# atenpas/gpd

Measured on NVIDIA H100. Metric: grasp candidates/sec end-to-end (15ch), higher is better.
Workload: dtype f64 geometry / f32 LeNet

## Files before the change

### gpd_b200/csrc/api.cu

```cuda
#include <atomic>
#include <cfloat>
#include <cmath>
#include <cstdarg>
#include <cstdio>
#include <cstdlib>
#include <cstring>
#include <string>
#include <vector>

#include "common.cuh"

static char g_create_err[512] = "";

struct StageTimes {
  struct Span { int stage; cudaEvent_t b, e; };
  std::vector<cudaEvent_t> pool;
  size_t used = 0;
  std::vector<Span> spans;
  cudaEvent_t get() {
    if (used == pool.size()) {
      cudaEvent_t e;
      cudaEventCreate(&e);
      pool.push_back(e);
    }
// ... 2117 lines not shown
        const int c = st.ecount[(size_t)r * B + b];
        if (eval_round_counts_out) eval_round_counts_out[(size_t)b * R + r] = c;
        if (eval_xyz_out) memcpy(eval_xyz_out + 3 * o, ev.data() + 3 * ((size_t)b * R + r) * S, sizeof(double) * 3 * c);
        o += c;
      }
      if (eval_offsets_out) eval_offsets_out[b + 1] = (int32_t)o;
    }
  }
  if (kept_offsets_out) memcpy(kept_offsets_out, st.koff.data(), sizeof(int32_t) * ((size_t)B + 1));
  if (kept_xyz_out)
    for (int b = 0; b < B; b++)
      memcpy(kept_xyz_out + 3 * (size_t)st.koff[b], kp.data() + 3 * ((size_t)st.init_off[b] + (size_t)b * RS),
             sizeof(double) * 3 * (size_t)(st.koff[b + 1] - st.koff[b]));
  return B;
}

void gpdb_free_result(gpdb_result *r) {
  if (!r) return;
  if (r->owner_) {
    HostArena *a = (HostArena *)r->owner_;
    a->in_use = false;
    arena_unref(a);
  } else {
    free(r->frame_valid);
    free(r->frames);
    free(r->pose_flags);
    free(r->pose_scores);
    free(r->candidates);
    free(r->images);
  }
  memset(r, 0, sizeof(*r));
}

int gpdb_debug_phase_cycles(gpdb_ctx *ctx, int enable, uint64_t cycles_out[16]) {
  if (!ctx) return GPDB_ERR_INVALID;
  CUDA_TRY(cudaSetDevice(ctx->device));
  CUDA_TRY(cudaStreamSynchronize(ctx->stream));
  if (ctx->d_prof && cycles_out)
    CUDA_TRY(cudaMemcpy(cycles_out, ctx->d_prof, sizeof(uint64_t) * 16, cudaMemcpyDeviceToHost));
  if (enable && !ctx->d_prof) CUDA_TRY(cudaMalloc(&ctx->d_prof, sizeof(uint64_t) * 32));
  if (enable) CUDA_TRY(cudaMemset(ctx->d_prof, 0, sizeof(uint64_t) * 32));
  if (!enable && ctx->d_prof) {
    cudaFree(ctx->d_prof);
    ctx->d_prof = nullptr;
  }
  return GPDB_OK;
}

int gpdb_debug_path_counts(gpdb_ctx *ctx, uint64_t counts_out[16]) {
  if (!ctx || !counts_out) return GPDB_ERR_INVALID;
  CUDA_TRY(cudaSetDevice(ctx->device));
  CUDA_TRY(cudaStreamSynchronize(ctx->stream));
  if (ctx->d_prof)
    CUDA_TRY(cudaMemcpy(counts_out, ctx->d_prof + GPDB_PROF_PATH, sizeof(uint64_t) * 16, cudaMemcpyDeviceToHost));
  else
    memset(counts_out, 0, sizeof(uint64_t) * 16);
  return GPDB_OK;
}

int gpdb_last_timings(const gpdb_ctx *ctx, double ms_out[8]) {
  if (!ctx || !ms_out) return GPDB_ERR_INVALID;
  for (int i = 0; i < 8; i++) ms_out[i] = ctx->last_ms[i];
  return GPDB_OK;
}

}
```

### gpd_b200/csrc/common.cuh

```cuda
#pragma once
#include <cuda_runtime.h>
#include <stdint.h>

#include "../../include/gpd_b200.h"
#include "../../include/gpd_b200_shadow.h"

#define GPDB_MAX_ORIENT 32
#define GPDB_MAX_SLOTS 32
#define GPDB_MAX_DEEPEN 64
#define GPDB_MAX_NSP 128

struct DevParams {
  double finger_width, hand_outer_diameter, hand_depth, hand_height, init_bite;
  int P, n_axes, n_orient, nfp;
  int axes[GPDB_MAX_HAND_AXES];
  int deepen, slots_disjoint, all_axes_z;
  double inv_slot_step;
  double fs[GPDB_MAX_SLOTS];
  double fsw[GPDB_MAX_SLOTS];
  int J;
  double topj[GPDB_MAX_DEEPEN], botj[GPDB_MAX_DEEPEN];
  double cosf;
  int min_viable;
  double min_ap, max_ap, ws[6];
// ... 41 lines not shown
struct CloudTable {
  const CloudDesc *d;
  const int *soff;
  int n;
};

struct CloudSet {
  float4 *pts4;
  float *xyz;
  double *nrm;
  uint8_t *cam;
  int *src;
  int *cell_start;
  CloudDesc *desc;
  int *soff;
  int *off;
  int *sel;
  int *pos;
  size_t point_cap, cell_cap, desc_cap;
  int n, maxk;
  bool has_src;
  double *samples;
  int n_samples;
  size_t samples_cap;
  int positions(int b) const { return n_samples ? pos[b + 1] - pos[b] : 0; }
  DevCloud view;
  int points() const { return n ? off[n] : 0; }
  CloudTable table() const { return CloudTable{desc, soff, n}; }
};

#define GPDB_NERR 8

#define GPDB_PROF_PATH 16
enum PathEvent {
  PATH_FRAMES_T1, PATH_FRAMES_T2, PATH_HANDS_T2, PATH_HANDS_T3, PATH_HANDS_SLAB, PATH_IMG2_BOX, PATH_IMG2_NONUNIT, PATH_IMG_GL,
  PATH_IMG2_CAST, PATH_IMG2_DRAW, PATH_IMG2_STASH, PATH_IMG_CAST, PATH_IMG_DRAW, PATH_IMG_STASH, PATH_IMG_BALL
};

#define CUDA_TRY(expr)                                                                        \
  do {                                                                                        \
    cudaError_t e__ = (expr);                                                                 \
    if (e__ != cudaSuccess) {                                                                 \
      gpdb_set_error(ctx, GPDB_ERR_CUDA, "%s:%d %s -> %s", __FILE__, __LINE__, #expr,         \
                     cudaGetErrorString(e__));                                                \
      return GPDB_ERR_CUDA;                                                                   \
    }                                                                                         \
  } while (0)

struct LenetWeights {
  float *c1w, *c1b, *c2w, *c2b, *i1w, *i1b, *i2w, *i2b;
  int C;
  bool set;
};

struct C1Affine {
  float scale[20], bias[20];
};
struct LenetTc {
  void *b1, *b2, *b3;
  C1Affine c1_aff;
  int npl, nch1;
  float w2_scale, a2_scale, w3_scale, x3_scale;
  bool ready;
};

struct StageTimes;
// ... 165 lines not shown
```

### gpd_b200/csrc/geometry.cu

```cuda
#include <cfloat>
#include <climits>
#include <cstdlib>
#include <vector>
#include <cub/cub.cuh>

#include "common.cuh"
#include "grid.cuh"

namespace {

constexpr int NT_HANDS = 256;
#ifndef GPDB_NT_IMG
#define GPDB_NT_IMG 512
#endif
constexpr int NT_IMG = GPDB_NT_IMG;
constexpr int LRF_WARPS = 4;
constexpr int LRF_CAP_GLOBAL = 16384;
constexpr int LRF_CAP = 1024;
constexpr int BOX_CAP = 2048;
constexpr int MAXPIX = 64 * 64;

__device__ __forceinline__ void to_frame(const double *F, double v0, double v1, double v2, double &o0, double &o1,
                                         double &o2) {
  o0 = (F[0] * v0 + F[1] * v1) + F[2] * v2;
// ... 1152 lines not shown
  }
  return !__any_sync(0xffffffffu, empty);
}
template <int NT>
__device__ __forceinline__ void occ_ballot(unsigned *occf, int t, bool occupied) {
  const unsigned word = __ballot_sync(0xffffffffu, occupied);
  if ((threadIdx.x & 31) == 0) occf[(threadIdx.x >> 5) + t * (NT / 32)] = word;
}

template <int NT>
__device__ __noinline__ float dilated_min(const float *F, int S) {
  float mn = FLT_MAX;
  for (int pix = threadIdx.x; pix < S * S; pix += NT) {
    const int r = pix / S, c = pix - r * S;
    float m = -FLT_MAX;
    for (int dr = -1; dr <= 1; dr++)
      for (int dc = -1; dc <= 1; dc++) {
        const int rr = r + dr, cc = c + dc;
        if (rr >= 0 && rr < S && cc >= 0 && cc < S) m = fmaxf(m, F[rr * S + cc]);
      }
    mn = fminf(mn, m);
  }
  return mn;
}

#define PHASE(i)                                                        \
  do {                                                                  \
    if (prof && threadIdx.x == 0) {                                     \
      long long now__ = clock64();                                      \
      if ((i) > 1) atomicAdd(prof + (i), (unsigned long long)(now__ - t_phase)); \
      t_phase = now__;                                                  \
    }                                                                   \
  } while (0)


__device__ __forceinline__ int warp_append(bool pred, int *counter) {
  const unsigned mk = __ballot_sync(0xffffffffu, pred);
  if (!mk) return 0;
  const int lane = threadIdx.x & 31, leader = __ffs(mk) - 1;
  int base = 0;
  if (lane == leader) base = atomicAdd(counter, __popc(mk));
  base = __shfl_sync(0xffffffffu, base, leader);
  return base + __popc(mk & ((1u << lane) - 1));
}

template <class R, class E>
__device__ __forceinline__ void warp_expand_bits(unsigned bits, unsigned code, R &&reserve, E &&emit) {
  const int lane = threadIdx.x & 31;
  const int cnt = __popc(bits);
  int incl = cnt;
#pragma unroll
  for (int o = 1; o < 32; o <<= 1) {
    const int v = __shfl_up_sync(0xffffffffu, incl, o);
    if (lane >= o) incl += v;
  }
  const int total = __shfl_sync(0xffffffffu, incl, 31);
  const int base = reserve(total);
  for (int j0 = 0; j0 < total; j0 += 32) {
    const int j = j0 + lane;
    int w = 0;
#pragma unroll
    for (int s = 16; s; s >>= 1) {
      const int v = __shfl_sync(0xffffffffu, incl, w + s - 1);
      if (v <= j) w += s;
    }
    const unsigned wbits = __shfl_sync(0xffffffffu, bits, w), wcode = __shfl_sync(0xffffffffu, code, w);
    const int wexcl = __shfl_sync(0xffffffffu, incl - cnt, w);
    if (j < total) emit(base + j, wcode | __fns(wbits, 0, j - wexcl + 1));
  }
}

template <class E>
__device__ __forceinline__ void expand_bitmap(const unsigned *bitmap, int nbits, int d1, int *counter, E &&emit) {
  const int lane = threadIdx.x & 31;
  for (int wd0 = 0; wd0 * 32 < nbits; wd0 += NT_IMG) {
    const int wd = wd0 + threadIdx.x;
    const unsigned bits = (wd * 32 < nbits) ? bitmap[wd] : 0u;
    const int rowi = wd >> 1;
    const unsigned code = ((unsigned)(rowi % d1) << 8) | ((unsigned)(rowi / d1) << 16) | ((unsigned)(wd & 1) << 5);
    warp_expand_bits(
        bits, code,
// ... 189 lines not shown
  bool nrm, dep;
};
template <class W>
__device__ __forceinline__ void winners_to_planes(const PointPlanes &pp, const float (&mnv)[2], const float (&mxv)[2],
                                                  bool background, W &&for_each_winner) {
  const Quant qn(mnv[0], mxv[0]), qd(mnv[1], mxv[1]);
  if (background) {
    const unsigned bg_n = qn(0.0f) * 0x01010101u, bg_d = qd(0.0f) * 0x01010101u;
    for (int k = threadIdx.x; k < (pp.plb >> 2); k += NT_IMG) {
      if (pp.nrm)
#pragma unroll
        for (int c = 0; c < 3; c++) reinterpret_cast<unsigned *>(pp.base + (size_t)(pp.cb + c) * pp.plb)[k] = bg_n;
      if (pp.dep) reinterpret_cast<unsigned *>(pp.base + (size_t)pp.cd * pp.plb)[k] = bg_d;
    }
    __syncthreads();
  }
  for_each_winner([&](int o, float n0, float n1, float n2, float dv) {
    if (pp.nrm) {
      pp.base[(size_t)(pp.cb + 0) * pp.plb + o] = (uint8_t)qn(n0);
      pp.base[(size_t)(pp.cb + 1) * pp.plb + o] = (uint8_t)qn(n1);
      pp.base[(size_t)(pp.cb + 2) * pp.plb + o] = (uint8_t)qn(n2);
    }
    if (pp.dep) pp.base[(size_t)pp.cd * pp.plb + o] = (uint8_t)qd(dv);
  });
}


template <class Sm, class G>
__device__ __noinline__ void shadow_setup(const DevParams &P, const G &Gd, Sm &sm, double gmax, unsigned *bitmap,
                                             int bm_total) {
  const gpdb_pose &h = sm.h;
  const int tid = threadIdx.x;
  const double voxel = GPDB_SHADOW_VOXEL;
  if (tid == 0) {
    const double jmax = gmax * voxel * 0.3 + 1e-9;
    const double half_od = P.vol_w / 2.0;
    double mn[3] = {DBL_MAX, DBL_MAX, DBL_MAX}, mx[3] = {-DBL_MAX, -DBL_MAX, -DBL_MAX};
    for (int cr = 0; cr < 8; cr++) {
      double cx = (cr & 1) ? h.bottom + P.vol_d : h.bottom;
      double cy = (cr & 2) ? h.center + half_od : h.center - half_od;
      double cz = (cr & 4) ? P.vol_h : -P.vol_h;
      for (int r = 0; r < 3; r++) {
        double wv = h.frame[r] * cx + h.frame[3 + r] * cy + h.frame[6 + r] * cz + h.sample[r];
        mn[r] = fmin(mn[r], wv);
        mx[r] = fmax(mx[r], wv);
      }
    }
    for (int r = 0; r < 3; r++) {
      int lo = (int)floor((mn[r] - jmax) * P.vox_mult) - 1;
      int hi = (int)floor((mx[r] + jmax) * P.vox_mult) + 1;
      sm.bm_org[r] = lo;
      sm.bm_dims[r] = min(hi - lo + 1, P.bm_dim);
    }
    for (int e = 0; e < 9; e++) sm.fR[e] = (float)h.frame[e];
    for (int r = 0; r < 3; r++) sm.fs[r] = (float)h.sample[r];
    const float jm = (float)(gmax * voxel * 0.3 * 1.7320508075688772 + 2e-5);
    sm.fbx_lo[0] = (float)h.bottom - jm;
    sm.fbx_lo[1] = (float)(h.center - P.vol_w / 2.0) - jm;
    sm.fbx_lo[2] = (float)(-P.vol_h) - jm;
    sm.fbx_hi[0] = (float)(h.bottom + P.vol_d) + jm;
    sm.fbx_hi[1] = (float)(h.center + P.vol_w / 2.0) + jm;
    sm.fbx_hi[2] = (float)P.vol_h + jm;
    const double wm = 0.0105;
    const double bx_lo[3] = {h.bottom - wm, h.center - P.vol_w / 2.0 - wm, -P.vol_h - wm};
    const double bx_hi[3] = {h.bottom + P.vol_d + wm, h.center + P.vol_w / 2.0 + wm, P.vol_h + wm};
    for (int a = 0; a < 3; a++) {
      sm.cull_lo[a] = (float)bx_lo[a] - 1e-5f;
      sm.cull_hi[a] = (float)bx_hi[a] + 1e-5f;
    }
  }
  if (tid < Gd.K) {
    double s0 = sm.center[0] - Gd.vp[tid][0], s1 = sm.center[1] - Gd.vp[tid][1], s2 = sm.center[2] - Gd.vp[tid][2];
    double nn = sqrt((s0 * s0 + s1 * s1) + s2 * s2);
    sm.sv[tid][0] = P.shadow_length * s0 / nn;
    sm.sv[tid][1] = P.shadow_length * s1 / nn;
    sm.sv[tid][2] = P.shadow_length * s2 / nn;
    double svh[3];
    to_frame(h.frame, sm.sv[tid][0], sm.sv[tid][1], sm.sv[tid][2], svh[0], svh[1], svh[2]);
    for (int a = 0; a < 3; a++) {
      const float dv = (float)svh[a];
      sm.cull_inv[tid][a] = fabsf(dv) < 1e-6f ? 0.0f : 1.0f / dv;
    }
  }
  for (int k = tid; k < bm_total; k += NT_IMG) bitmap[k] = 0u;
}

struct VoxelBox {
  int o0, o1, o2, d0, d1, d2;
  template <class Sm>
  __device__ __forceinline__ explicit VoxelBox(const Sm &sm)
      : o0(sm.bm_org[0]), o1(sm.bm_org[1]), o2(sm.bm_org[2]), d0(sm.bm_dims[0]), d1(sm.bm_dims[1]), d2(sm.bm_dims[2]) {}
};

__device__ __forceinline__ bool voxel_point_in_box(const DevParams &P, const gpdb_pose &h, const double *qtab, int v0, int v1,
                                                   int v2, double &x, double &y, double &z) {
  const double voxel = GPDB_SHADOW_VOXEL;
  double g = qtab[gpdb_voxel_hash(v0, v1, v2) & (GPDB_QTAB_SIZE - 1)];
  double jit = 1.0 * g * voxel * 0.3;
  double w0 = (double)v0 * voxel + jit, w1 = (double)v1 * voxel + jit, w2 = (double)v2 * voxel + jit;
  to_frame(h.frame, w0 - h.sample[0], w1 - h.sample[1], w2 - h.sample[2], x, y, z);
  return in_image_box(P, h, x, y, z);
}
// ... 32 lines not shown
  float tmin = 0.0f, tmax = 1.0f;
  bool hit = true;
#pragma unroll
  for (int a = 0; a < 3; a++) {
    if (cull_inv[a] == 0.0f) {
      hit = hit && o3[a] >= sm.cull_lo[a] && o3[a] <= sm.cull_hi[a];
    } else {
      const float t1 = (sm.cull_lo[a] - o3[a]) * cull_inv[a], t2 = (sm.cull_hi[a] - o3[a]) * cull_inv[a];
      tmin = fmaxf(tmin, fminf(t1, t2));
      tmax = fminf(tmax, fmaxf(t1, t2));
    }
  }
  if (!hit || tmin > tmax) return false;
  const int r0 = max((int)floorf(tmin * 32767.0f) - 1, 0), r1 = min((int)ceilf(tmax * 32767.0f) + 1, 32767);
  rg = (unsigned)r0 | ((unsigned)r1 << 16);
  return true;
}

struct CastLists {
  float4 *wl;
  unsigned *wrange;
  int wl_cap;
  unsigned *dlist;
  int dl_cap;
  int path_cast, path_draw;
};

template <class Sm, class G, class BallAt>
__device__ __forceinline__ void cast_camera(const DevParams &P, const G &Gd, const DevCloud &cl, const SegRange &sr,
                                            const float (&q)[3], Sm &sm, const VoxelBox &vb, int k, unsigned *bm,
                                            const CastLists &L, bool use_ball, int nball, BallAt &&ball_at,
                                            unsigned long long *prof, bool count_walks) {
  const int tid = threadIdx.x;
  __syncthreads();
  if (tid == 0) {
    sm.wl_n = 0;
    sm.dl_n = 0;
  }
  __syncthreads();
  auto append = [&](bool ok, const float4 &p, unsigned rg) {
    const int pos = warp_append(ok, &sm.wl_n);
    if (!ok) return;
    const unsigned seed0 = gpdb_shadow_seed((unsigned)sm.h.sample_index, (unsigned)__float_as_int(p.w), (unsigned)k);
    if (pos < L.wl_cap) {
      L.wl[pos] = make_float4(p.x, p.y, p.z, __uint_as_float(seed0));
      L.wrange[pos] = rg;
    } else {
      unsigned seed = seed0;
      const int r0 = (int)(rg & 0xFFFFu), r1 = (int)(rg >> 16);
      for (int t = 0; t < P.nsp; t++) {
        int r = (int)gpdb_fastrand(&seed);
        if (r >= r0 && r <= r1) set_bit(bm, draw_bit(P, sm, vb, (double)p.x, (double)p.y, (double)p.z, seed, k));
      }
    }
  };
  if (use_ball) {
    for (int i0 = 0; i0 < nball; i0 += NT_IMG) {
      const int i = i0 + tid;
      float4 p = make_float4(0.f, 0.f, 0.f, 0.f);
      unsigned rg = 0;
      bool ok = false;
      if (i < nball) {
        p = __ldg(cl.pts4 + ball_at(i));
        ok = cull(sm, k, p, rg);
      }
      append(ok, p, rg);
    }
  } else {
    scan_balanced<NT_IMG>(Gd, cl, sr, sm.seg, [&](bool in, const float4 &p, int) {
      unsigned rg = 0;
      const bool ok = in && l2_simple(q, p.x, p.y, p.z) < P.r2_img && cull(sm, k, p, rg);
      append(ok, p, rg);
    });
    if (count_walks && prof && tid == 0) atomicAdd(prof + 14, 1ull);
  }
  __syncthreads();
  const int nw = min(sm.wl_n, L.wl_cap);
  if (prof && tid == 0) {
    atomicAdd(prof + 9, (unsigned long long)nw);
    if (sm.wl_n > L.wl_cap) atomicAdd(prof + GPDB_PROF_PATH + L.path_cast, (unsigned long long)(sm.wl_n - L.wl_cap));
  }
  const int nsp = P.nsp;
  const unsigned nsp_magic = nsp > 1 ? (unsigned)((0x100000000ull + (unsigned)nsp - 1) / (unsigned)nsp) : 0u;
  const int nd = nw * nsp;
  for (int w0 = 0; w0 < nd; w0 += NT_IMG) {
    const int w = w0 + tid;
    bool pass = false;
    unsigned code = 0, seed = 0;
    if (w < nd) {
      const int item = nsp > 1 ? (int)__umulhi((unsigned)w, nsp_magic) : w, t = w - item * nsp;
      seed = sm.lcgA[t] * __float_as_uint(L.wl[item].w) + sm.lcgC[t];
      const unsigned rg = L.wrange[item];
      const int r = (int)((seed >> 16) & 0x7FFFu);
      pass = r >= (int)(rg & 0xFFFFu) && r <= (int)(rg >> 16);
      code = ((unsigned)item << 7) | (unsigned)t;
    }
    const int pos = warp_append(pass, &sm.dl_n);
    if (pass) {
      if (pos < L.dl_cap) L.dlist[pos] = code;
      else {
        const float4 e = L.wl[code >> 7];
        set_bit(bm, draw_bit(P, sm, vb, (double)e.x, (double)e.y, (double)e.z, seed, k));
      }
    }
  }
  __syncthreads();
  const int ndl = min(sm.dl_n, L.dl_cap);
  if (prof && tid == 0) {
    atomicAdd(prof + 10, (unsigned long long)sm.dl_n);
    if (sm.dl_n > L.dl_cap) atomicAdd(prof + GPDB_PROF_PATH + L.path_draw, (unsigned long long)(sm.dl_n - L.dl_cap));
  }
  auto list_bit = [&](int i) -> int {
    if (i >= ndl) return -1;
    const unsigned code = L.dlist[i];
    const float4 e = L.wl[code >> 7];
    const int t = (int)(code & 127u);
    const unsigned seed = sm.lcgA[t] * __float_as_uint(e.w) + sm.lcgC[t];
    return draw_bit(P, sm, vb, (double)e.x, (double)e.y, (double)e.z, seed, k);
  };
  for (int i = tid; i < ndl; i += 2 * NT_IMG) {
    const int bit_a = list_bit(i), bit_b = list_bit(i + NT_IMG);
    set_bit(bm, bit_a);
    set_bit(bm, bit_b);
  }
}

__device__ __forceinline__ void intersect_bitmaps(unsigned *bitmap, int bm_words, int K, int cam_set) {
  if (K < 2) return;
  for (int wd = threadIdx.x; wd < bm_words; wd += NT_IMG) {
    unsigned acc = bitmap[wd];
    for (int k = 1; k < K; k++)
      if ((cam_set >> k) & 1) acc &= bitmap[(size_t)k * bm_words + wd];
    bitmap[wd] = acc;
  }
}

__device__ __forceinline__ uint2 eval_voxel(const DevParams &P, const gpdb_pose &h, const double *qtab, const double (&inv)[3],
                                            int S, const VoxelBox &vb, unsigned long long *tiles, unsigned code, int pj_lo,
                                            int pj_hi) {
  int b0 = code & 255, b1 = (code >> 8) & 255, b2 = code >> 16;
  double x, y, z;
  if (!voxel_point_in_box(P, h, qtab, b0 + vb.o0, b1 + vb.o1, b2 + vb.o2, x, y, z)) return make_uint2(0u, 0u);
  double u[3];
  int cellv[3];
  unit_cells(P, h, inv, S, x, y, z, u, cellv);
  uint2 st = make_uint2(0u, 0u);
#pragma unroll
  for (int pj = 0; pj < 3; pj++) {
    const Proj pr(pj);
    const int pix = (S - 1 - cellv[pr.a0]) * S + cellv[pr.a1];
    const unsigned qv = unit_q32(u[pr.a2]);
    if (pj >= pj_lo && pj < pj_hi) cell_add(tiles + (size_t)(pj - pj_lo) * S * S + pix, qv);
    if (pj == 2) st = make_uint2((unsigned)pix | 0x80000000u, qv);
  }
  return st;
}

template <class Sm>
__device__ __forceinline__ void shadow_channel(Sm &sm, const double *rcp, int S, unsigned long long *tile, uint8_t *plane,
                                               int rs) {
  constexpr int PIXT = (MAXPIX + NT_IMG - 1) / NT_IMG;
  const int tid = threadIdx.x, SS = S * S;
  float avgr[PIXT];
  unsigned occm = 0;
  float mm[2] = {-FLT_MAX, -FLT_MAX};
#pragma unroll
  for (int t = 0; t < PIXT; t++) {
    const int pix = tid + t * NT_IMG;
    avgr[t] = 0.0f;
    bool oc = false;
    if (pix < SS) {
      const unsigned long long acc = tile[pix];
      const unsigned cntc = (unsigned)(acc >> 48);
      if (cntc) {
        avgr[t] = (float)cell_mean(acc, rcp);
        occm |= 1u << t;
        oc = true;
        mm[0] = fmaxf(mm[0], avgr[t]);
        mm[1] = fmaxf(mm[1], -avgr[t]);
      }
    }
    if (t * NT_IMG < SS) occ_ballot<NT_IMG>(sm.occf, t, oc);
  }
  bool covered;
  block_max<NT_IMG, 2>(mm, sm.fred, sm.occf, S, &covered);
// ... 291 lines not shown
      const int nset = min(sm.wl_n, BL_CAP);
      if (prof && tid == 0) {
        atomicAdd(prof + 11, (unsigned long long)sm.wl_n);
        atomicAdd(prof + 12, (unsigned long long)bn);
        atomicAdd(prof + 13, (unsigned long long)sm.n_img);
        if (sm.wl_n > BL_CAP) atomicAdd(prof + GPDB_PROF_PATH + PATH_IMG_STASH, 1ull);
        if (sm.ball_n > BALL_CAP) atomicAdd(prof + GPDB_PROF_PATH + PATH_IMG_BALL, 1ull);
      }
      for (int i = tid; i < nset; i += NT_IMG) eval_voxel(P, h, qtab, inv, S, vb, tileA, blist[i], 0, 3);
      __syncthreads();
      PHASE(6);
      for (int pj = 0; pj < 3; pj++) shadow_channel(sm, rcp, S, tileA + (size_t)pj * SS, planes + (size_t)(pj * 5 + 4) * PLB, RS);
      __syncthreads();
      for (int k = tid; k < MAXPIX / 32; k += NT_IMG) sm.occf[k] = 0u;
    }
    __syncthreads();
    PHASE(7);
    dilate_assemble(S, RS >> 2, C, [&](int ch) { return planes + (size_t)ch * PLB; }, reinterpret_cast<uint4 *>(p16) + (size_t)b * SS);
    PHASE(8);
  }
}

constexpr int BOX_CAP2 = 1024;
constexpr int IMG2_S = 60;
constexpr int BALL_CAP2 = (IMG2_S * IMG2_S * 16 - 12 * IMG2_S * IMG2_S) / 4;
using Img2Smem = ImgSmemT<2>;
constexpr size_t IMG2_DYN_SMEM = (size_t)2 * 8 * IMG2_S * IMG2_S + (size_t)3 * IMG2_S * IMG2_S + (size_t)BOX_CAP2 * 36;
static_assert(2 * (IMG2_DYN_SMEM + sizeof(Img2Smem) + 1024) <= 228 * 1024, "k_images2 no longer fits two CTAs per SM");

template <bool BATCH>
__global__ void __launch_bounds__(NT_IMG, 2) k_images2(const DevParams *Pp, DevCloud cl0, CloudTable tab, const gpdb_pose *cand, int nc,
                                                       uint8_t *p16, const double *qtab, int *ovf, int *ovf_count,
                                                       unsigned long long *prof) {
  long long t_phase = 0;
  const DevParams &P = *Pp;
  extern __shared__ __align__(16) unsigned char dyn[];
  __shared__ Img2Smem sm;
  constexpr int S = IMG2_S, SS = S * S, RW = S / 4, PLB = SS;
  constexpr int JW = (BOX_CAP2 + NT_IMG - 1) / NT_IMG;
  const int C = P.C;
  unsigned long long *tileA = reinterpret_cast<unsigned long long *>(dyn);
  unsigned long long *tileB = tileA + SS;
  uint8_t *splanes = reinterpret_cast<uint8_t *>(tileB + SS);
  unsigned char *lbase = splanes + 3 * PLB;
  constexpr int LIST_BYTES = BOX_CAP2 * 36;
  const BoxList bl(lbase, BOX_CAP2);
  unsigned *bitmap = reinterpret_cast<unsigned *>(lbase);
  uint8_t *tplanes = reinterpret_cast<uint8_t *>(tileA);
  const int tid = threadIdx.x;
  const int nproj = (C >= 12) ? 3 : 1;
  const bool do_nrm = C != 1, do_dep = C == 1 || C >= 12;
  const int npp = (C == 15 || C == 12) ? 12 : C;
  img_cta_init(sm, P);

  for (int b = blockIdx.x; b < nc; b += gridDim.x) {
    img_begin(sm, cand + b);
    uint8_t *gimg = p16 + (size_t)b * SS * 16;
    int *ball = reinterpret_cast<int *>(gimg + 12 * PLB);
    for (int k = tid; k < (npp * PLB) >> 4; k += NT_IMG) reinterpret_cast<uint4 *>(gimg)[k] = make_uint4(0, 0, 0, 0);
    for (int k = tid; k < SS; k += NT_IMG) reinterpret_cast<uint4 *>(tileA)[k] = make_uint4(0, 0, 0, 0);
    for (int k = tid; k < (3 * PLB) >> 4; k += NT_IMG) reinterpret_cast<uint4 *>(splanes)[k] = make_uint4(0, 0, 0, 0);
    __syncthreads();
    PHASE(1);
    const gpdb_pose &h = sm.h;
    const auto &G = CloudSel<BATCH>::get(tab, h.sample_slot);
    const DevCloud cl = CloudSel<BATCH>::local(G, cl0);
    const double inv[3] = {1.0 / P.vol_d, 1.0 / P.vol_w, 1.0 / (2.0 * P.vol_h)};
// ... 65 lines not shown
        for (int j = 0; j < JW; j++)
          if (wpix[j] >= 0) emit(wpix[j], wv[j][0], wv[j][1], wv[j][2], wv[j][3]);
      });
      if (covered) {
        for (int k = tid; k < SS; k += NT_IMG) reinterpret_cast<uint4 *>(tileA)[k] = make_uint4(0, 0, 0, 0);
        for (int k = tid; k < MAXPIX / 32; k += NT_IMG) sm.occf[k] = 0u;
      } else {
        __syncthreads();
        wipe_cells(bl, bn, S, pr, tileA, tileB, sm.occf);
      }
      __syncthreads();
    }
    PHASE(3);

    if (C == 15) {
      const int K = G.K, bm_words = 2 * P.bm_dim * P.bm_dim;
      shadow_setup(P, G, sm, qtab[GPDB_QTAB_SIZE - 1], bitmap, bm_words * K);
      __syncthreads();
      PHASE(4);
      const VoxelBox vb(sm);
      const int cam_set = sm.cam_or, nball = sm.ball_n;
      float4 *wl = reinterpret_cast<float4 *>(tileA);
      constexpr int WL_CAP = (SS * 8) / 20;
      const CastLists L = {wl, reinterpret_cast<unsigned *>(wl + WL_CAP), WL_CAP, reinterpret_cast<unsigned *>(tileB), 2 * SS,
                           PATH_IMG2_CAST, PATH_IMG2_DRAW};
      for (int k = 0; k < K; k++) {
        if (!((cam_set >> k) & 1)) continue;
        cast_camera(P, G, cl, sr, q, sm, vb, k, bitmap + (size_t)k * bm_words, L, nball <= BALL_CAP2, nball,
                    [&](int i) { return __ldcg(ball + i); },
                    prof, true);
      }
      __syncthreads();
      PHASE(5);
      intersect_bitmaps(bitmap, bm_words, K, cam_set);
      for (int k = tid; k < SS; k += NT_IMG) reinterpret_cast<uint4 *>(tileA)[k] = make_uint4(0, 0, 0, 0);
      if (tid == 0) sm.wl_n = 0;
      __syncthreads();
      const int nbits = 64 * vb.d1 * vb.d2;
      uint2 *stash = reinterpret_cast<uint2 *>(bitmap + (((size_t)bm_words * (K > 1 ? K : 1) + 1) & ~(size_t)1));
      const int ST_CAP = (LIST_BYTES - (int)((reinterpret_cast<unsigned char *>(stash)) - lbase)) / 8;
      expand_bitmap(bitmap, nbits, vb.d1, &sm.wl_n, [&](int pos, unsigned code) {
        if (pos < ST_CAP) stash[pos].x = code;
        else eval_voxel(P, h, qtab, inv, S, vb, tileA, code, 0, 2);
      });
      __syncthreads();
      const int nset_all = sm.wl_n, nset = min(nset_all, ST_CAP);
      if (prof && tid == 0) {
        atomicAdd(prof + 11, (unsigned long long)nset_all);
        atomicAdd(prof + 12, (unsigned long long)bn);
        atomicAdd(prof + 13, (unsigned long long)sm.n_img);
        if (nset_all > ST_CAP) atomicAdd(prof + GPDB_PROF_PATH + PATH_IMG2_STASH, 1ull);
      }
      for (int i = tid; i < nset; i += NT_IMG) stash[i] = eval_voxel(P, h, qtab, inv, S, vb, tileA, stash[i].x, 0, 2);
      __syncthreads();
      PHASE(6);
      shadow_channel(sm, rcp, S, tileA, splanes, S);
      shadow_channel(sm, rcp, S, tileB, splanes + PLB, S);
      __syncthreads();
      for (int k = tid; k < SS / 2; k += NT_IMG) reinterpret_cast<uint4 *>(tileA)[k] = make_uint4(0, 0, 0, 0);
      __syncthreads();
      if (nset_all <= ST_CAP) {
        for (int i = tid; i < nset; i += NT_IMG) {
          const uint2 st = stash[i];
          if (st.x & 0x80000000u) {
            const bool carry = cell_add(tileA + (st.x & 0x7fffffffu), st.y);
            if (prof && carry) atomicAdd(prof + 0, 1ull);
          }
        }
      } else {
        expand_bitmap(bitmap, nbits, vb.d1, nullptr, [&](int, unsigned code) { eval_voxel(P, h, qtab, inv, S, vb, tileA, code, 2, 3); });
      }
      __syncthreads();
      if (prof) {
        unsigned most = 0;
        for (int k = tid; k < SS; k += NT_IMG) most = max(most, (unsigned)(tileA[k] >> 48));
        most = __reduce_max_sync(0xffffffffu, most);
        if ((tid & 31) == 0 && most) atomicMax(prof + 1, (unsigned long long)most);
      }
      shadow_channel(sm, rcp, S, tileA, splanes + 2 * PLB, S);
      __syncthreads();
      for (int k = tid; k < MAXPIX / 32; k += NT_IMG) sm.occf[k] = 0u;
    }
    __syncthreads();
    PHASE(7);
    for (int k = tid; k < (npp * PLB) >> 4; k += NT_IMG)
      reinterpret_cast<uint4 *>(tplanes)[k] = __ldcg(reinterpret_cast<const uint4 *>(gimg) + k);
    __syncthreads();
    dilate_assemble(S, RW, C, [&](int ch) {
      return (C == 15) ? ((ch % 5 == 4) ? splanes + (size_t)(ch / 5) * PLB : tplanes + (size_t)(4 * (ch / 5) + ch % 5) * PLB)
                       : tplanes + (size_t)ch * PLB;
    }, reinterpret_cast<uint4 *>(gimg));
    PHASE(8);
  }
}

__global__ void k_p16_to_hwc(const uint8_t *__restrict__ p16, size_t npix, int C, uint8_t *__restrict__ hwc) {
  const size_t i = (size_t)blockIdx.x * blockDim.x + threadIdx.x;
  if (i >= npix * (size_t)C) return;
  const size_t pix = i / C;
  hwc[i] = p16[pix * 16 + (i - pix * C)];
}
__global__ void k_hwc_to_p16(const uint8_t *__restrict__ hwc, size_t npix, int C, uint8_t *__restrict__ p16) {
  const size_t i = (size_t)blockIdx.x * blockDim.x + threadIdx.x;
  if (i >= npix) return;
  unsigned w[4] = {0u, 0u, 0u, 0u};
  for (int c = 0; c < C; c++) w[c >> 2] |= (unsigned)hwc[i * C + c] << (8 * (c & 3));
  reinterpret_cast<uint4 *>(p16)[i] = make_uint4(w[0], w[1], w[2], w[3]);
}

__global__ void k_batch_desc(const int *bounds, CloudDesc *d, int B, long long *ncell) {
  const int b = blockIdx.x * blockDim.x + threadIdx.x;
  if (b >= B) return;
  CloudDesc &D = d[b];
  float lo[3], hi[3];
  for (int a = 0; a < 3; a++) {
    const int mn = bounds[6 * b + a], mx = bounds[6 * b + 3 + a];
// ... 435 lines not shown
```

### gpd_b200/lib.py

```python
import ctypes as C
import os

import numpy as np

from . import abi

_HERE = os.path.dirname(os.path.abspath(__file__))
SO_PATH = os.environ.get("GPD_B200_LIB") or os.path.join(_HERE, "libgpd_b200.so")
_LIB = None

EXPORTS = [
    "gpdb_params_default", "gpdb_create", "gpdb_destroy", "gpdb_last_error", "gpdb_load_weights_dir",
    "gpdb_set_weights", "gpdb_set_cloud", "gpdb_detect", "gpdb_frames", "gpdb_hand_search", "gpdb_images",
    "gpdb_classify", "gpdb_free_result", "gpdb_last_timings", "gpdb_build_info", "gpdb_detect_resident",
    "gpdb_set_stream", "gpdb_debug_phase_cycles", "gpdb_preprocess_params_default", "gpdb_preprocess",
    "gpdb_get_cloud", "gpdb_get_cloud_source_index", "gpdb_preprocess_timings", "gpdb_detect_select", "gpdb_load_weights_file", "gpdb_read_weights_file", "gpdb_set_samples",
    "gpdb_comm_unique_id", "gpdb_comm_init", "gpdb_comm_destroy", "gpdb_shard_bounds", "gpdb_set_cloud_bcast",
    "gpdb_detect_sharded", "gpdb_detect_sharded_resident", "gpdb_slot_bytes", "gpdb_find_clusters", "gpdb_reevaluate", "gpdb_set_overlap",
    "gpdb_set_clouds", "gpdb_detect_batch", "gpdb_detect_batch_select", "gpdb_preprocess_clouds", "gpdb_get_clouds",
    "gpdb_debug_path_counts", "gpdb_debug_lenet_layers", "gpdb_set_clouds_samples", "gpdb_hand_search_batch",
    "gpdb_find_clusters_batch", "gpdb_preprocess_clouds_device", "gpdb_set_clouds_device", "gpdb_detect_batch_select_device",
    "gpdb_find_clusters_batch_device", "gpdb_sis_params_default", "gpdb_sis_batch", "gpdb_sis_batch_device",
    "gpdb_sis_positions",
]
# ... 617 lines not shown
        sidx = np.ascontiguousarray(sample_idx, dtype=np.int32)
        n = len(sidx)
        frames = np.zeros((n, 9))
        valid = np.zeros(n, np.uint8)
        self._check(lib().gpdb_frames(self.h, _p(sidx), n, _p(frames), _p(valid)))
        return frames, valid

    def images(self, poses):
        poses = np.ascontiguousarray(poses, dtype=abi.POSE_DTYPE)
        n = len(poses)
        S, Cc = self.params.image_size, self.params.image_num_channels
        out = np.zeros((n, S, S, Cc), np.uint8)
        self._check(lib().gpdb_images(self.h, _p(poses), n, _p(out)))
        return out

    def classify(self, images):
        images = np.ascontiguousarray(images, dtype=np.uint8)
        n = images.shape[0]
        scores = np.zeros(n, np.float32)
        logits = np.zeros((n, 2), np.float32)
        self._check(lib().gpdb_classify(self.h, _p(images), n, _p(scores), _p(logits)))
        return scores, logits

    def lenet_layers(self, images):
        images = np.ascontiguousarray(images, dtype=np.uint8)
        n = images.shape[0]
        out = {"pool1": np.zeros((n, 20, 28, 28), np.float32), "pool2": np.zeros((n, 7200), np.float64),
               "ip1": np.zeros((n, 500), np.float32), "logits": np.zeros((n, 2), np.float32)}
        self._check(lib().gpdb_debug_lenet_layers(self.h, _p(images), n, _p(out["pool1"]), _p(out["pool2"]), _p(out["ip1"]),
                                                  _p(out["logits"])))
        return out

    def phase_cycles(self, enable=1):
        out = np.zeros(16, np.uint64)
        self._check(lib().gpdb_debug_phase_cycles(self.h, enable, _p(out)))
        return out

    def path_counts(self):
        out = np.zeros(16, np.uint64)
        self._check(lib().gpdb_debug_path_counts(self.h, _p(out)))
        return {name: int(out[i]) for i, name in enumerate(PATH_EVENTS)}

    def last_timings(self):
        ms = np.zeros(8)
        lib().gpdb_last_timings(self.h, _p(ms))
        return ms


def comm_unique_id():
    buf = C.create_string_buffer(128)
    rc = lib().gpdb_comm_unique_id(buf)
    if rc != 0:
        raise GpdbError(rc, lib().gpdb_last_error(None).decode())
    return buf.raw


def shard_bounds(n, rank, nranks):
    lo, hi, st = C.c_int32(), C.c_int32(), C.c_int32()
    lib().gpdb_shard_bounds(int(n), int(rank), int(nranks), C.byref(lo), C.byref(hi), C.byref(st))
    return lo.value, hi.value, st.value


def slot_bytes(slot_samples, P):
    return int(lib().gpdb_slot_bytes(int(slot_samples), int(P)))


def free_result(res):
# ... 2 lines not shown
```

### include/gpd_b200.h

```cpp
#ifndef GPD_B200_H_
#define GPD_B200_H_

#include <stdint.h>

#ifdef __cplusplus
extern "C" {
#endif

#define GPDB_VERSION 1

#define GPDB_OK 0
#define GPDB_ERR_INVALID (-1)
#define GPDB_ERR_CUDA (-2)
#define GPDB_ERR_STATE (-3)
#define GPDB_ERR_IO (-4)
#define GPDB_ERR_CAPACITY (-5)

#define GPDB_MAX_CAMERAS 8
#define GPDB_MAX_HAND_AXES 3

#define GPDB_POSE_VALID 1u
#define GPDB_POSE_FILTERED 2u
#define GPDB_POSE_HALF 4u
#define GPDB_POSE_FULL 8u
// ... 190 lines not shown
  double prob_rand_samples;
  double standard_deviation;
  int32_t sampling_method;
  double workspace[6];
  double min_score;
  int32_t min_inliers;
  uint64_t seed;
} gpdb_sis_params;

void gpdb_sis_params_default(gpdb_sis_params *p);

int gpdb_sis_batch(gpdb_ctx *ctx, const gpdb_sis_params *sp, const int32_t *init_offsets, const int32_t *init_idx,
                   gpdb_result *out, int32_t *hand_offsets_out);
int gpdb_sis_batch_device(gpdb_ctx *ctx, const gpdb_sis_params *sp, const int32_t *init_offsets, const int32_t *d_init_idx,
                          gpdb_pose *d_hands_out, int32_t *hand_offsets_out, gpdb_result *stats);
int gpdb_sis_positions(gpdb_ctx *ctx, int32_t *eval_offsets_out, int32_t *eval_round_counts_out, double *eval_xyz_out,
                       int32_t *kept_offsets_out, double *kept_xyz_out);

void gpdb_free_result(gpdb_result *r);

#define GPDB_COMM_ID_BYTES 128
int gpdb_comm_unique_id(char id_out[GPDB_COMM_ID_BYTES]);
int gpdb_comm_init(gpdb_ctx *ctx, const char id[GPDB_COMM_ID_BYTES], int32_t rank, int32_t nranks);
int gpdb_comm_destroy(gpdb_ctx *ctx);
void gpdb_shard_bounds(int32_t n, int32_t rank, int32_t nranks, int32_t *lo, int32_t *hi, int32_t *slot_samples);
int gpdb_set_cloud_bcast(gpdb_ctx *ctx, int32_t root, const float *xyz, const double *normals, const int32_t *cam_source,
                         int32_t n_points, const double *view_points, int32_t n_cams);
int gpdb_detect_sharded(gpdb_ctx *ctx, const int32_t *sample_idx, int32_t n_samples, gpdb_result *out);
int gpdb_detect_sharded_resident(gpdb_ctx *ctx, const int32_t *d_sample_idx_local, int32_t n_local, int32_t slot_samples,
                                 uint8_t *d_gathered, gpdb_result *stats);
int64_t gpdb_slot_bytes(int32_t slot_samples, int32_t poses_per_sample);

int gpdb_last_timings(const gpdb_ctx *ctx, double ms_out[8]);
int gpdb_debug_phase_cycles(gpdb_ctx *ctx, int enable, uint64_t cycles_out[16]);
int gpdb_debug_path_counts(gpdb_ctx *ctx, uint64_t counts_out[16]);
int gpdb_debug_lenet_layers(gpdb_ctx *ctx, const uint8_t *images_hwc, int32_t n, float *pool1_out, double *pool2_out,
                            float *ip1_out, float *logits_out);

const char *gpdb_build_info(void);

#ifdef __cplusplus
}
#endif
#endif
```

Measured before the change: 1.887 million.

## Parallelize image setup, batch window filtering, spill stash to global, add sub-phase profiling

Computes the per-candidate bounding box across a warp with shuffles instead of a single thread. Drops one barrier by moving the wl_n reset earlier. Processes four window draws per thread with a single warp scan and atomic. Adds an early exit to warp_expand_bits when a warp has no set bits. Extends the voxel stash into the global ball buffer so fewer poses fall back to re-expansion. It also adds sub-phase clock profiling and conflict counters that only run when profiling is enabled. The global spill adds memory traffic, and the recomputed seed in the overflow path must match the original draw.

Result: faster. 1.985 million, median of 6 (+5.2%).

```diff
diff --git a/gpd_b200/csrc/api.cu b/gpd_b200/csrc/api.cu
--- a/gpd_b200/csrc/api.cu
+++ b/gpd_b200/csrc/api.cu
@@ -2173,14 +2173,16 @@
   memset(r, 0, sizeof(*r));
 }
 
-int gpdb_debug_phase_cycles(gpdb_ctx *ctx, int enable, uint64_t cycles_out[16]) {
+int gpdb_debug_phase_cycles(gpdb_ctx *ctx, int enable, uint64_t cycles_out[32]) {
   if (!ctx) return GPDB_ERR_INVALID;
   CUDA_TRY(cudaSetDevice(ctx->device));
   CUDA_TRY(cudaStreamSynchronize(ctx->stream));
-  if (ctx->d_prof && cycles_out)
+  if (ctx->d_prof && cycles_out) {
     CUDA_TRY(cudaMemcpy(cycles_out, ctx->d_prof, sizeof(uint64_t) * 16, cudaMemcpyDeviceToHost));
-  if (enable && !ctx->d_prof) CUDA_TRY(cudaMalloc(&ctx->d_prof, sizeof(uint64_t) * 32));
-  if (enable) CUDA_TRY(cudaMemset(ctx->d_prof, 0, sizeof(uint64_t) * 32));
+    CUDA_TRY(cudaMemcpy(cycles_out + 16, ctx->d_prof + GPDB_PROF_SUB, sizeof(uint64_t) * 16, cudaMemcpyDeviceToHost));
+  }
+  if (enable && !ctx->d_prof) CUDA_TRY(cudaMalloc(&ctx->d_prof, sizeof(uint64_t) * GPDB_PROF_SLOTS));
+  if (enable) CUDA_TRY(cudaMemset(ctx->d_prof, 0, sizeof(uint64_t) * GPDB_PROF_SLOTS));
   if (!enable && ctx->d_prof) {
     cudaFree(ctx->d_prof);
     ctx->d_prof = nullptr;
diff --git a/gpd_b200/csrc/common.cuh b/gpd_b200/csrc/common.cuh
--- a/gpd_b200/csrc/common.cuh
+++ b/gpd_b200/csrc/common.cuh
@@ -97,6 +97,8 @@
 #define GPDB_NERR 8
 
 #define GPDB_PROF_PATH 16
+#define GPDB_PROF_SUB 32
+#define GPDB_PROF_SLOTS 48
 enum PathEvent {
   PATH_FRAMES_T1, PATH_FRAMES_T2, PATH_HANDS_T2, PATH_HANDS_T3, PATH_HANDS_SLAB, PATH_IMG2_BOX, PATH_IMG2_NONUNIT, PATH_IMG_GL,
   PATH_IMG2_CAST, PATH_IMG2_DRAW, PATH_IMG2_STASH, PATH_IMG_CAST, PATH_IMG_DRAW, PATH_IMG_STASH, PATH_IMG_BALL
diff --git a/gpd_b200/csrc/geometry.cu b/gpd_b200/csrc/geometry.cu
--- a/gpd_b200/csrc/geometry.cu
+++ b/gpd_b200/csrc/geometry.cu
@@ -1208,6 +1208,14 @@
       t_phase = now__;                                                  \
     }                                                                   \
   } while (0)
+__device__ __forceinline__ void sub_phase(unsigned long long *prof, int i, long long &t) {
+  if (prof && threadIdx.x == 0) {
+    const long long now = clock64();
+    atomicAdd(prof + GPDB_PROF_SUB + i, (unsigned long long)(now - t));
+    t = now;
+  }
+}
+enum SubPhase { SUB_CULL, SUB_WINDOW, SUB_EXPAND, SUB_CHANNELS, SUB_STASH, SUB_CLEARS, SUB_PROBE, SUB_EVT_SHARED };
 
 
 __device__ __forceinline__ int warp_append(bool pred, int *counter) {
@@ -1223,6 +1231,7 @@
 template <class R, class E>
 __device__ __forceinline__ void warp_expand_bits(unsigned bits, unsigned code, R &&reserve, E &&emit) {
   const int lane = threadIdx.x & 31;
+  if (!__any_sync(0xffffffffu, bits != 0u)) return;
   const int cnt = __popc(bits);
   int incl = cnt;
 #pragma unroll
@@ -1478,42 +1487,42 @@
   const gpdb_pose &h = sm.h;
   const int tid = threadIdx.x;
   const double voxel = GPDB_SHADOW_VOXEL;
-  if (tid == 0) {
-    const double jmax = gmax * voxel * 0.3 + 1e-9;
+  if (tid < 32) {
     const double half_od = P.vol_w / 2.0;
-    double mn[3] = {DBL_MAX, DBL_MAX, DBL_MAX}, mx[3] = {-DBL_MAX, -DBL_MAX, -DBL_MAX};
-    for (int cr = 0; cr < 8; cr++) {
+    double wv = 0.0;
+    if (tid < 24) {
+      const int cr = tid / 3, r = tid - 3 * cr;
       double cx = (cr & 1) ? h.bottom + P.vol_d : h.bottom;
       double cy = (cr & 2) ? h.center + half_od : h.center - half_od;
       double cz = (cr & 4) ? P.vol_h : -P.vol_h;
-      for (int r = 0; r < 3; r++) {
-        double wv = h.frame[r] * cx + h.frame[3 + r] * cy + h.frame[6 + r] * cz + h.sample[r];
-        mn[r] = fmin(mn[r], wv);
-        mx[r] = fmax(mx[r], wv);
-      }
-    }
-    for (int r = 0; r < 3; r++) {
-      int lo = (int)floor((mn[r] - jmax) * P.vox_mult) - 1;
-      int hi = (int)floor((mx[r] + jmax) * P.vox_mult) + 1;
-      sm.bm_org[r] = lo;
-      sm.bm_dims[r] = min(hi - lo + 1, P.bm_dim);
-    }
-    for (int e = 0; e < 9; e++) sm.fR[e] = (float)h.frame[e];
-    for (int r = 0; r < 3; r++) sm.fs[r] = (float)h.sample[r];
-    const float jm = (float)(gmax * voxel * 0.3 * 1.7320508075688772 + 2e-5);
-    sm.fbx_lo[0] = (float)h.bottom - jm;
-    sm.fbx_lo[1] = (float)(h.center - P.vol_w / 2.0) - jm;
-    sm.fbx_lo[2] = (float)(-P.vol_h) - jm;
-    sm.fbx_hi[0] = (float)(h.bottom + P.vol_d) + jm;
-    sm.fbx_hi[1] = (float)(h.center + P.vol_w / 2.0) + jm;
-    sm.fbx_hi[2] = (float)P.vol_h + jm;
-    const double wm = 0.0105;
-    const double bx_lo[3] = {h.bottom - wm, h.center - P.vol_w / 2.0 - wm, -P.vol_h - wm};
-    const double bx_hi[3] = {h.bottom + P.vol_d + wm, h.center + P.vol_w / 2.0 + wm, P.vol_h + wm};
-    for (int a = 0; a < 3; a++) {
-      sm.cull_lo[a] = (float)bx_lo[a] - 1e-5f;
-      sm.cull_hi[a] = (float)bx_hi[a] + 1e-5f;
-    }
+      wv = h.frame[r] * cx + h.frame[3 + r] * cy + h.frame[6 + r] * cz + h.sample[r];
+    }
+    double mn = DBL_MAX, mx = -DBL_MAX;
+#pragma unroll
+    for (int cr = 0; cr < 8; cr++) {
+      const double v = __shfl_sync(0xffffffffu, wv, 3 * cr + tid % 3);
+      mn = fmin(mn, v);
+      mx = fmax(mx, v);
+    }
+    if (tid < 3) {
+      const int a = tid;
+      const double jmax = gmax * voxel * 0.3 + 1e-9;
+      int lo = (int)floor((mn - jmax) * P.vox_mult) - 1;
+      int hi = (int)floor((mx + jmax) * P.vox_mult) + 1;
+      sm.bm_org[a] = lo;
+      sm.bm_dims[a] = min(hi - lo + 1, P.bm_dim);
+      sm.fs[a] = (float)h.sample[a];
+      const float jm = (float)(gmax * voxel * 0.3 * 1.7320508075688772 + 2e-5);
+      sm.fbx_lo[a] = (a == 0 ? (float)h.bottom : a == 1 ? (float)(h.center - P.vol_w / 2.0) : (float)(-P.vol_h)) - jm;
+      sm.fbx_hi[a] = (a == 0 ? (float)(h.bottom + P.vol_d) : a == 1 ? (float)(h.center + P.vol_w / 2.0) : (float)P.vol_h) + jm;
+      const double wm = 0.0105;
+      const double bx_lo = a == 0 ? h.bottom - wm : a == 1 ? h.center - P.vol_w / 2.0 - wm : -P.vol_h - wm;
+      const double bx_hi = a == 0 ? h.bottom + P.vol_d + wm : a == 1 ? h.center + P.vol_w / 2.0 + wm : P.vol_h + wm;
+      sm.cull_lo[a] = (float)bx_lo - 1e-5f;
+      sm.cull_hi[a] = (float)bx_hi + 1e-5f;
+    }
+    if (tid < 9) sm.fR[tid] = (float)h.frame[tid];
+    if (tid == 0) sm.wl_n = 0;
   }
   if (tid < Gd.K) {
     double s0 = sm.center[0] - Gd.vp[tid][0], s1 = sm.center[1] - Gd.vp[tid][1], s2 = sm.center[2] - Gd.vp[tid][2];
@@ -1612,12 +1621,10 @@
                                             const CastLists &L, bool use_ball, int nball, BallAt &&ball_at,
                                             unsigned long long *prof, bool count_walks) {
   const int tid = threadIdx.x;
+  long long t_sub = 0;
+  if (prof && tid == 0) t_sub = clock64();
   __syncthreads();
-  if (tid == 0) {
-    sm.wl_n = 0;
-    sm.dl_n = 0;
-  }
-  __syncthreads();
+  if (tid == 0) sm.dl_n = 0;
   auto append = [&](bool ok, const float4 &p, unsigned rg) {
     const int pos = warp_append(ok, &sm.wl_n);
     if (!ok) return;
@@ -1655,6 +1662,7 @@
     if (count_walks && prof && tid == 0) atomicAdd(prof + 14, 1ull);
   }
   __syncthreads();
+  sub_phase(prof, SUB_CULL, t_sub);
   const int nw = min(sm.wl_n, L.wl_cap);
   if (prof && tid == 0) {
     atomicAdd(prof + 9, (unsigned long long)nw);
@@ -1663,29 +1671,50 @@
   const int nsp = P.nsp;
   const unsigned nsp_magic = nsp > 1 ? (unsigned)((0x100000000ull + (unsigned)nsp - 1) / (unsigned)nsp) : 0u;
   const int nd = nw * nsp;
-  for (int w0 = 0; w0 < nd; w0 += NT_IMG) {
-    const int w = w0 + tid;
-    bool pass = false;
-    unsigned code = 0, seed = 0;
-    if (w < nd) {
-      const int item = nsp > 1 ? (int)__umulhi((unsigned)w, nsp_magic) : w, t = w - item * nsp;
-      seed = sm.lcgA[t] * __float_as_uint(L.wl[item].w) + sm.lcgC[t];
-      const unsigned rg = L.wrange[item];
-      const int r = (int)((seed >> 16) & 0x7FFFu);
-      pass = r >= (int)(rg & 0xFFFFu) && r <= (int)(rg >> 16);
-      code = ((unsigned)item << 7) | (unsigned)t;
-    }
-    const int pos = warp_append(pass, &sm.dl_n);
-    if (pass) {
-      if (pos < L.dl_cap) L.dlist[pos] = code;
+  constexpr int WT = 4;
+  const int lane = tid & 31;
+  for (int w0 = 0; w0 < nd; w0 += WT * NT_IMG) {
+    unsigned code[WT], pm = 0;
+#pragma unroll
+    for (int j = 0; j < WT; j++) {
+      const int w = w0 + j * NT_IMG + tid;
+      code[j] = 0;
+      if (w < nd) {
+        const int item = nsp > 1 ? (int)__umulhi((unsigned)w, nsp_magic) : w, t = w - item * nsp;
+        const unsigned seed = sm.lcgA[t] * __float_as_uint(L.wl[item].w) + sm.lcgC[t];
+        const unsigned rg = L.wrange[item];
+        const int r = (int)((seed >> 16) & 0x7FFFu);
+        if (r >= (int)(rg & 0xFFFFu) && r <= (int)(rg >> 16)) pm |= 1u << j;
+        code[j] = ((unsigned)item << 7) | (unsigned)t;
+      }
+    }
+    const int cnt = __popc(pm);
+    int incl = cnt;
+#pragma unroll
+    for (int o = 1; o < 32; o <<= 1) {
+      const int v = __shfl_up_sync(0xffffffffu, incl, o);
+      if (lane >= o) incl += v;
+    }
+    int pos = 0;
+    if (lane == 31 && incl) pos = atomicAdd(&sm.dl_n, incl);
+    pos = __shfl_sync(0xffffffffu, pos, 31) + incl - cnt;
+#pragma unroll
+    for (int j = 0; j < WT; j++) {
+      if (!((pm >> j) & 1u)) continue;
+      if (pos < L.dl_cap) L.dlist[pos] = code[j];
       else {
-        const float4 e = L.wl[code >> 7];
+        const float4 e = L.wl[code[j] >> 7];
+        const int t = (int)(code[j] & 127u);
+        const unsigned seed = sm.lcgA[t] * __float_as_uint(e.w) + sm.lcgC[t];
         set_bit(bm, draw_bit(P, sm, vb, (double)e.x, (double)e.y, (double)e.z, seed, k));
       }
+      pos++;
     }
   }
   __syncthreads();
+  sub_phase(prof, SUB_WINDOW, t_sub);
   const int ndl = min(sm.dl_n, L.dl_cap);
+  if (tid == 0) sm.wl_n = 0;
   if (prof && tid == 0) {
     atomicAdd(prof + 10, (unsigned long long)sm.dl_n);
     if (sm.dl_n > L.dl_cap) atomicAdd(prof + GPDB_PROF_PATH + L.path_draw, (unsigned long long)(sm.dl_n - L.dl_cap));
@@ -1717,7 +1746,7 @@
 
 __device__ __forceinline__ uint2 eval_voxel(const DevParams &P, const gpdb_pose &h, const double *qtab, const double (&inv)[3],
                                             int S, const VoxelBox &vb, unsigned long long *tiles, unsigned code, int pj_lo,
-                                            int pj_hi) {
+                                            int pj_hi, unsigned long long *evt = nullptr) {
   int b0 = code & 255, b1 = (code >> 8) & 255, b2 = code >> 16;
   double x, y, z;
   if (!voxel_point_in_box(P, h, qtab, b0 + vb.o0, b1 + vb.o1, b2 + vb.o2, x, y, z)) return make_uint2(0u, 0u);
@@ -1730,7 +1759,10 @@
     const Proj pr(pj);
     const int pix = (S - 1 - cellv[pr.a0]) * S + cellv[pr.a1];
     const unsigned qv = unit_q32(u[pr.a2]);
-    if (pj >= pj_lo && pj < pj_hi) cell_add(tiles + (size_t)(pj - pj_lo) * S * S + pix, qv);
+    if (pj >= pj_lo && pj < pj_hi) {
+      if (evt && __popc(__match_any_sync(__activemask(), pj * S * S + pix)) > 1) atomicAdd(evt, 1ull);
+      cell_add(tiles + (size_t)(pj - pj_lo) * S * S + pix, qv);
+    }
     if (pj == 2) st = make_uint2((unsigned)pix | 0x80000000u, qv);
   }
   return st;
@@ -2088,7 +2120,7 @@
 __global__ void __launch_bounds__(NT_IMG, 2) k_images2(const DevParams *Pp, DevCloud cl0, CloudTable tab, const gpdb_pose *cand, int nc,
                                                        uint8_t *p16, const double *qtab, int *ovf, int *ovf_count,
                                                        unsigned long long *prof) {
-  long long t_phase = 0;
+  long long t_phase = 0, t_sub = 0;
   const DevParams &P = *Pp;
   extern __shared__ __align__(16) unsigned char dyn[];
   __shared__ Img2Smem sm;
@@ -2220,18 +2252,27 @@
       }
       __syncthreads();
       PHASE(5);
+      t_sub = t_phase;
       intersect_bitmaps(bitmap, bm_words, K, cam_set);
       for (int k = tid; k < SS; k += NT_IMG) reinterpret_cast<uint4 *>(tileA)[k] = make_uint4(0, 0, 0, 0);
       if (tid == 0) sm.wl_n = 0;
       __syncthreads();
       const int nbits = 64 * vb.d1 * vb.d2;
       uint2 *stash = reinterpret_cast<uint2 *>(bitmap + (((size_t)bm_words * (K > 1 ? K : 1) + 1) & ~(size_t)1));
-      const int ST_CAP = (LIST_BYTES - (int)((reinterpret_cast<unsigned char *>(stash)) - lbase)) / 8;
+      const int ST_SM = (LIST_BYTES - (int)((reinterpret_cast<unsigned char *>(stash)) - lbase)) / 8;
+      uint2 *gstash = reinterpret_cast<uint2 *>(ball);
+      const int ST_CAP = ST_SM + BALL_CAP2 / 2;
+      auto st_put = [&](int i, uint2 v) {
+        if (i < ST_SM) stash[i] = v;
+        else __stcg(gstash + (i - ST_SM), v);
+      };
+      auto st_get = [&](int i) -> uint2 { return i < ST_SM ? stash[i] : __ldcg(gstash + (i - ST_SM)); };
       expand_bitmap(bitmap, nbits, vb.d1, &sm.wl_n, [&](int pos, unsigned code) {
-        if (pos < ST_CAP) stash[pos].x = code;
+        if (pos < ST_CAP) st_put(pos, make_uint2(code, 0u));
         else eval_voxel(P, h, qtab, inv, S, vb, tileA, code, 0, 2);
       });
       __syncthreads();
+      sub_phase(prof, SUB_EXPAND, t_sub);
       const int nset_all = sm.wl_n, nset = min(nset_all, ST_CAP);
       if (prof && tid == 0) {
         atomicAdd(prof + 11, (unsigned long long)nset_all);
@@ -2239,18 +2280,23 @@
         atomicAdd(prof + 13, (unsigned long long)sm.n_img);
         if (nset_all > ST_CAP) atomicAdd(prof + GPDB_PROF_PATH + PATH_IMG2_STASH, 1ull);
       }
-      for (int i = tid; i < nset; i += NT_IMG) stash[i] = eval_voxel(P, h, qtab, inv, S, vb, tileA, stash[i].x, 0, 2);
+      unsigned long long *evt = prof ? prof + GPDB_PROF_SUB + SUB_EVT_SHARED : nullptr;
+      for (int i = tid; i < nset; i += NT_IMG) st_put(i, eval_voxel(P, h, qtab, inv, S, vb, tileA, st_get(i).x, 0, 2, evt));
       __syncthreads();
       PHASE(6);
+      t_sub = t_phase;
       shadow_channel(sm, rcp, S, tileA, splanes, S);
       shadow_channel(sm, rcp, S, tileB, splanes + PLB, S);
       __syncthreads();
+      sub_phase(prof, SUB_CHANNELS, t_sub);
       for (int k = tid; k < SS / 2; k += NT_IMG) reinterpret_cast<uint4 *>(tileA)[k] = make_uint4(0, 0, 0, 0);
       __syncthreads();
+      sub_phase(prof, SUB_CLEARS, t_sub);
       if (nset_all <= ST_CAP) {
         for (int i = tid; i < nset; i += NT_IMG) {
-          const uint2 st = stash[i];
+          const uint2 st = st_get(i);
           if (st.x & 0x80000000u) {
+            if (evt && __popc(__match_any_sync(__activemask(), st.x)) > 1) atomicAdd(evt, 1ull);
             const bool carry = cell_add(tileA + (st.x & 0x7fffffffu), st.y);
             if (prof && carry) atomicAdd(prof + 0, 1ull);
           }
@@ -2259,17 +2305,21 @@
         expand_bitmap(bitmap, nbits, vb.d1, nullptr, [&](int, unsigned code) { eval_voxel(P, h, qtab, inv, S, vb, tileA, code, 2, 3); });
       }
       __syncthreads();
+      sub_phase(prof, SUB_STASH, t_sub);
       if (prof) {
         unsigned most = 0;
         for (int k = tid; k < SS; k += NT_IMG) most = max(most, (unsigned)(tileA[k] >> 48));
         most = __reduce_max_sync(0xffffffffu, most);
         if ((tid & 31) == 0 && most) atomicMax(prof + 1, (unsigned long long)most);
       }
+      sub_phase(prof, SUB_PROBE, t_sub);
       shadow_channel(sm, rcp, S, tileA, splanes + 2 * PLB, S);
       __syncthreads();
+      sub_phase(prof, SUB_CHANNELS, t_sub);
       for (int k = tid; k < MAXPIX / 32; k += NT_IMG) sm.occf[k] = 0u;
     }
     __syncthreads();
+    if (C == 15) sub_phase(prof, SUB_CLEARS, t_sub);
     PHASE(7);
     for (int k = tid; k < (npp * PLB) >> 4; k += NT_IMG)
       reinterpret_cast<uint4 *>(tplanes)[k] = __ldcg(reinterpret_cast<const uint4 *>(gimg) + k);
diff --git a/gpd_b200/lib.py b/gpd_b200/lib.py
--- a/gpd_b200/lib.py
+++ b/gpd_b200/lib.py
@@ -673,7 +673,7 @@
         return out
 
     def phase_cycles(self, enable=1):
-        out = np.zeros(16, np.uint64)
+        out = np.zeros(32, np.uint64)
         self._check(lib().gpdb_debug_phase_cycles(self.h, enable, _p(out)))
         return out
 
diff --git a/include/gpd_b200.h b/include/gpd_b200.h
--- a/include/gpd_b200.h
+++ b/include/gpd_b200.h
@@ -246,7 +246,7 @@
 int64_t gpdb_slot_bytes(int32_t slot_samples, int32_t poses_per_sample);
 
 int gpdb_last_timings(const gpdb_ctx *ctx, double ms_out[8]);
-int gpdb_debug_phase_cycles(gpdb_ctx *ctx, int enable, uint64_t cycles_out[16]);
+int gpdb_debug_phase_cycles(gpdb_ctx *ctx, int enable, uint64_t cycles_out[32]);
 int gpdb_debug_path_counts(gpdb_ctx *ctx, uint64_t counts_out[16]);
 int gpdb_debug_lenet_layers(gpdb_ctx *ctx, const uint8_t *images_hwc, int32_t n, float *pool1_out, double *pool2_out,
                             float *ip1_out, float *logits_out);
```
